# yukara-ikemiya/world-class

Measured on AMD Instinct MI355X. Metric: analysis+synthesis frames/sec (whole node), 48 kHz 5 ms hop, higher is better.
Workload: dtype f64; 1 GPU; 64 synthetic 48 kHz 10 s utterances per GPU (8 distinct, tiled), 5 ms hop, Harvest->CheapTrick->D4C->Synthesis, inputs resident in HBM when the clock starts (`value`; SURVEY.md section 8(d)'s headline with H2D of x and D2H of all outputs inside the clock is `value_with_transfers`); utterances_per_gpu=64, frames_per_gpu=128064, fs=48000, fft_size=2048, parallelism=utterance-sharded x1 (shard.partition), final RCCL all-gather of F0 + checksums

## Files before the change

### world_class_amd/csrc/wc_stages.hpp

```cpp
#pragma once
#include <utility>
#include <vector>

#include "wc_internal.hpp"
#include "wc_stretch.hpp"

inline bool fft_size_supported(int fft_size) { return fft_size == 512 || fft_size == 1024 || fft_size == 2048 || fft_size == 4096; }

int hv_enqueue(wc_harvest *h, hipStream_t s, int n_utt, const double *d_x, const int *x_length, double *d_tpos, double *d_f0,
			   bool full, hipEvent_t mid_event, hipEvent_t start_after, int part = 3, hipEvent_t bp_done = nullptr,
			   hipEvent_t tail_after = nullptr);
int hv_overflowed(wc_harvest *h, hipStream_t s, bool *overflow, bool *tie = nullptr, std::vector<int> *tie_utts = nullptr);
std::vector<std::pair<int, int>> hv_runs_of(const std::vector<int> &us);
wc_harvest *hv_exact_twin(wc_harvest *h);
void hv_set_phases(wc_harvest *h, int mask);
int hv_row_width(const wc_harvest *h);
int hv_reserve_rows(wc_harvest *h, long long total_1ms_frames);
double *hv_candidate_rows(wc_harvest *h);
double *hv_score_rows(wc_harvest *h);

int ct_prepare(wc_cheaptrick *c, hipStream_t s, int n_utt, const int *x_length, const double *d_f0, const int *f0_length,
			   const uint64_t *rng_pos, long long *total_out, uint64_t *min_pos_out, uint64_t *max_end_out);
int ct_frames(wc_cheaptrick *c, hipStream_t s, int n_utt, const double *d_x, const double *d_tpos, const double *d_f0,
			  double *d_sp, long long total, hipEvent_t *rows_done);
// ... 5 lines not shown
				const double *d_f0, const int *f0_length, int fft_size, double *d_ap, const uint64_t *rng_pos,
				const unsigned long long *d_start);
const unsigned long long *d4c_end_positions(const wc_d4c *d);
uint64_t d4c_draw_bound(const wc_d4c *d, int f0_length);

int syn_prepare(wc_synthesis *sy, hipStream_t s, int n_utt, const double *d_f0, const int *f0_length, const int *out_length,
				double *d_out, const uint64_t *rng_pos, bool full);
int syn_pulses(wc_synthesis *sy, hipStream_t s, const double *d_f0, const double *d_sp, const double *d_ap, double *d_out,
			   const unsigned long long *d_start);
int syn_finish(wc_synthesis *sy, hipStream_t s, uint64_t *rng_pos_out, bool *overflow);

wc::Device *hv_device(const wc_harvest *h);
wc::Device *ct_device(const wc_cheaptrick *c);
wc::Device *d4c_device(const wc_d4c *d);
wc::Device *syn_device(const wc_synthesis *sy);
const double *syn_dc_remover(const wc_synthesis *sy);
int syn_fs(const wc_synthesis *sy);

namespace wc {
struct CodecPlanArgs {
	const int *k;
	const double *s;
	const double2 *w;
};
struct CodecPlan {
	DevBuf k, s, w, kp, sp;
	CodecPlanArgs args() const { return {k.as<int>(), s.as<double>(), w.as<double2>()}; }
	CodecPlanArgs wave_args() const { return {kp.as<int>(), sp.as<double>(), w.as<double2>()}; }
};
int codec_plan(Device *dev, int fs, int fft_size, bool coding, const CodecPlan **out);
// ... 35 lines not shown
```

### world_class_amd/csrc/wc_synth_stream.hip

```cpp
#include <algorithm>
#include <cfloat>
#include <climits>
#include <cmath>
#include <cstring>
#include <vector>

#include "wc_stages.hpp"
#include "wc_synthesis.hpp"
#include "../../include/world_class_codec.h"
#include "../../include/world_class_stream.h"

namespace wc {

struct SsDesc {
	long long win_old, win_new;
	long long in_off;
	int keep_from, keep, n_in;
	int f_base, f_len;
	int n0, n1;
	int cap;
	int has_pend, pend_idx, pend_vuv;
	double pend_shift;
	double run, wrap, vu;
	long long inc_off, slot;
// ... 181 lines not shown
	bool formed = false;
	double last = 0.0;
	long long src = 0;
	int cside = 0;
};
}

struct wc_synth_stream {
	int fs, fft_size, n_streams, max_frames, fp_ms_x1000;
	double frame_period;
	int gap, wcap, ccap, wsz;
	Device *dev;
	wc_synthesis *sy;
	std::vector<SsState> st;
	int parity = 0;
	DevBuf wf0[2], wsp[2], wap[2], carry[2], work, inc, pulses, resp, meta, owner, aux;
	DevBuf dsp, dap;
	DevBuf dmod, sf0;
	DevBuf cf0, csp, cap, rf0, rsp, rap, drt;
	DevBuf tf0, tcsp, tcap;
	HostBuf h_stage, h_mod, h_rt;
};

namespace {
struct SynthStreamGuard {
	wc_synth_stream *s;
	std::vector<SsState> st;
	int parity;
	bool keep = false;
	explicit SynthStreamGuard(wc_synth_stream *x) : s(x), st(x->st), parity(x->parity) {}
	~SynthStreamGuard() {
// ... 83 lines not shown
	const double spf = s->frame_period * fs;
	s->wcap = max_frames_per_push + (int)std::ceil((s->gap + fft_size + 2.0 * spf) / spf) + 8;
	s->ccap = s->gap + fft_size + 64;
	s->wsz = (int)((max_frames_per_push + 2) * std::ceil(spf)) + s->gap + fft_size + 64;
	s->st.assign(n_streams, SsState());
	return s;
}

void wc_synth_stream_destroy(wc_synth_stream *s) {
	if (!s) return;
	s->dev->quiesce();
	for (int k = 0; k < 2; ++k) { s->wf0[k].release(); s->wsp[k].release(); s->wap[k].release(); s->carry[k].release(); }
	s->dsp.release(); s->dap.release(); s->dmod.release(); s->sf0.release(); s->h_mod.release();
	s->cf0.release(); s->csp.release(); s->cap.release(); s->rf0.release(); s->rsp.release(); s->rap.release(); s->drt.release(); s->h_rt.release();
	s->tf0.release(); s->tcsp.release(); s->tcap.release();
	s->work.release(); s->inc.release(); s->pulses.release(); s->resp.release(); s->meta.release(); s->owner.release(); s->aux.release(); s->h_stage.release();
	wc_synthesis_destroy(s->sy);
	delete s;
}

int wc_synth_stream_max_samples_per_push(const wc_synth_stream *s) { return s ? s->wsz : WC_ERR_INVALID; }

int wc_synth_stream_reset(wc_synth_stream *s, int u) {
	if (!s || u < 0 || u >= s->n_streams) return fail(WC_ERR_INVALID, "synthesis stream: bad stream index");
	DeviceLock lock(s->dev);
	s->st[u] = SsState();
	return WC_OK;
}

unsigned long long wc_synth_stream_rng_position(const wc_synth_stream *s, int u) {
	return (s && u >= 0 && u < s->n_streams) ? s->st[u].rng_pos : 0ull;
// ... 269 lines not shown
		SynArgs sa;
		std::memset(&sa, 0, sizeof(sa));
		sa.utts = d_utt; sa.n_utt = na; sa.pulse_prefix = d_prefix; sa.cap_off = d_capoff; sa.first_index = d_first; sa.p = pb;
		sa.f0 = s->wf0[1 - par].as<double>(); sa.sp = s->wsp[1 - par].as<double>(); sa.ap = s->wap[1 - par].as<double>();
		sa.tw = s->dev->twiddle; sa.dc_remover = syn_dc_remover(s->sy);
		sa.out = atomic ? s->work.as<double>() : nullptr;
		sa.resp = atomic ? nullptr : s->resp.as<double>();
		sa.rng_start = nullptr; sa.trace = nullptr; sa.only_pulse = -1; sa.fs = s->fs; sa.frame_period = s->frame_period;
		std::vector<int> owner((size_t)total_p);
		for (int a = 0; a < na; ++a) std::fill(owner.begin() + prefix[a], owner.begin() + prefix[a + 1], a);
		DevBuf &pu = s->owner;
		if ((rc = pu.reserve(sizeof(int) * (size_t)total_p * 2))) return rc;
		WC_HIP(hipMemcpyAsync(pu.p, owner.data(), sizeof(int) * (size_t)total_p, hipMemcpyHostToDevice, hs));
		WC_HIP(hipMemsetAsync(pu.as<int>() + total_p, 0, sizeof(int) * (size_t)total_p, hs));
		WC_HIP(hipStreamSynchronize(hs));
		if (atomic) {
			std::vector<OlDesc> ex(ol);
			for (auto &d : ex) { d.dst_off = d.src_off / s->ccap * s->wsz; d.cut = d.lo; }
			ol_expand = ex;
		}
		uint64_t lo = ~0ull, hi = 0;
		for (int a = 0; a < na; ++a) {
			if (n_syn[a] == 0) continue;
			lo = std::min<uint64_t>(lo, start[a]);
			hi = std::max<uint64_t>(hi, start[a] + (uint64_t)(E[act[a]] - first[a]) + 1);
		}
		if (atomic) {
			if ((rc = s->aux.reserve(sizeof(OlDesc) * na))) return rc;
			WC_HIP(hipMemcpyAsync(s->aux.p, ol_expand.data(), sizeof(OlDesc) * na, hipMemcpyHostToDevice, hs));
			overlap(nullptr, carry_old, s->work.as<double>(), s->aux.as<OlDesc>());
			WC_HIP(hipStreamSynchronize(hs));
		}
		if (hi - lo <= (1ull << 28)) {
			if ((rc = s->dev->ensure_rng(lo, hi))) return rc;
			sa.rng_table = s->dev->rng_table.as<uint32_t>(); sa.rng_base = s->dev->rng_base;
			sa.pulse_utt = pu.as<int>();
			sa.total_pulses = total_p;
			if ((rc = syn_launch_responses(N, sa, hs))) return rc;
		} else {
			for (int a = 0; a < na; ++a) {
				if (n_syn[a] == 0) continue;
				if ((rc = s->dev->ensure_rng(start[a], start[a] + (uint64_t)(E[act[a]] - first[a]) + 1))) return rc;
				SynArgs one = sa;
				one.utts = d_utt + a; one.n_utt = 1; one.pulse_prefix = d_pairs + 2 * a; one.cap_off = d_capoff + a; one.first_index = d_first + a;
				one.rng_table = s->dev->rng_table.as<uint32_t>(); one.rng_base = s->dev->rng_base;
				one.pulse_utt = pu.as<int>() + total_p;
				one.resp = atomic ? nullptr : s->resp.as<double>() + prefix[a] * N;
				one.total_pulses = n_syn[a];
				if ((rc = syn_launch_responses(N, one, hs))) return rc;
				WC_HIP(hipStreamSynchronize(hs));
			}
		}
	}
	if (atomic && total_p > 0) {
		std::vector<OlDesc> sp(ol);
		for (auto &d : sp) { d.src_off = d.src_off / s->ccap * s->wsz; d.src_len = d.hi - d.lo; d.n_p = 0; }
		if ((rc = s->h_stage.reserve(meta_bytes))) return rc;
		std::memcpy(s->h_stage.p, sp.data(), sizeof(OlDesc) * na);
		WC_HIP(hipMemcpyAsync(d_ol, s->h_stage.p, sizeof(OlDesc) * na, hipMemcpyHostToDevice, hs));
		if ((rc = s->h_stage.mark(hs))) return rc;
		overlap(nullptr, s->work.as<double>(), carry_new, d_ol);
	} else {
		overlap(atomic ? nullptr : s->resp.as<double>(), carry_old, carry_new, d_ol);
// ... 280 lines not shown
```

### world_class_amd/csrc/wc_synthesis.hip

```cpp
#include <cmath>
#include <cstdlib>
#include <cstring>
#include <vector>

#include "wc_device.hpp"
#include "wc_internal.hpp"
#include "wc_frames.hpp"
#include "wc_wavefft.hpp"
#include "wc_hostcopy.hpp"
#include "wc_synthesis.hpp"
#include "wc_stages.hpp"

namespace wc {

constexpr double kSafe = 0.000000000001;

struct TbArgs {
	const UttDesc *utts;
	const double *f0;
	const long long *cap_off;
	const int *cap;
	PulseBuf p;
	int *count;
	int *first_index;
// ... 1024 lines not shown
	wf_r2c_unpack(mr, mi, nyq, tw, lane);
#pragma unroll
	for (int s = 0; s < 16; ++s) {
		const double t = wf_exp_l(mr[s] * (0.5 / N), T);
		double sn, cs;
		wf_sincos(mi[s] * (0.5 / N), sn, cs);
		mr[s] = t * cs;
		mi[s] = t * sn;
	}
	mMr = wf_exp_l(nyq * (0.5 / N), T);
}

#ifndef WC_SYN_WAVE_OCC
#define WC_SYN_WAVE_OCC 2
#endif
#ifndef WC_SYN_ROWS_G
#define WC_SYN_ROWS_G 2
#endif
#ifndef WC_SYN_PARK_NOISE
#define WC_SYN_PARK_NOISE 1
#endif
#ifndef WC_SYN_ROW_PF
#define WC_SYN_ROW_PF 0
#endif
#ifndef WC_SYN_TRACE
#define WC_SYN_TRACE 0
#endif
#if WC_SYN_TRACE
#define SYN_STAMP(i) do { if (lane == 0) a.trace[gp * 16 + (i)] = __builtin_readcyclecounter(); } while (0)
#else
#define SYN_STAMP(i) do { } while (0)
#endif
template <bool ATOMIC>
__global__ __launch_bounds__(64) __attribute__((amdgpu_waves_per_eu(WC_SYN_WAVE_OCC, WC_SYN_WAVE_OCC))) void syn_pulse_wave_kernel(SynArgs a) {
	constexpr int N = 2048, M = 1024;
	__shared__ __attribute__((aligned(16))) double L[kWfLds];
	__shared__ __attribute__((aligned(16))) double T[kWfTabLds];
#if WC_SYN_PARK_NOISE
	__shared__ __attribute__((aligned(16))) double P[1024];
#endif
	const int lane = threadIdx.x;
#ifdef WC_SYN_LDS_PAD
	__shared__ double PAD[WC_SYN_LDS_PAD];
	if (a.fs < 0) PAD[lane] = 0.0;
#endif
	const long long total_p = a.pulse_prefix[a.n_utt];
	if ((long long)blockIdx.x >= 8 * ((total_p + 7) / 8)) return;
	const long long gp = xcd_frame(blockIdx.x, total_p);
	if (gp >= total_p) return;
	if (a.only_pulse >= 0 && gp != a.only_pulse) return;
	const int u = a.pulse_utt[gp];
	wf_tables_to_lds(T, a.tw, lane);
	const UttDesc ud = a.utts[u];
	const long long slot = a.cap_off[u] + (gp - a.pulse_prefix[u]);
	const int pidx = a.p.index[slot];
	const double shift = a.p.shift[slot];
	const int noise_size = a.p.noise_size[slot];
	const double vuv = (double)a.p.vuv[slot];
	const int fs = a.fs, Lf = ud.f_len;
	const double fp = a.frame_period;
	const double t = pidx / (double)fs;

	const int fl = min(Lf - 1, (int)floor(t / fp));
	const int ce = min(Lf - 1, (int)ceil(t / fp));
	const double ipol = uniform_d(t / fp - fl);
	const double *__restrict__ sf = a.sp + (ud.f_off + fl - ud.f_base) * (long long)(M + 1);
	const double *__restrict__ sc = a.sp + (ud.f_off + ce - ud.f_base) * (long long)(M + 1);
	const double *__restrict__ af = a.ap + (ud.f_off + fl - ud.f_base) * (long long)(M + 1);
	const double *__restrict__ ac = a.ap + (ud.f_off + ce - ud.f_base) * (long long)(M + 1);
	const bool same = fl == ce;
	auto blend = [&](double s0, double s1, double a0, double a1, double &env, double &ar) {
		if (same) {
			env = fabs(s0);
			const double s = safe_ap(a0);
			ar = s * s;
		} else {
			env = fma(1.0 - ipol, fabs(s0), ipol * fabs(s1));
			const double s = (1.0 - ipol) * safe_ap(a0) + ipol * safe_ap(a1);
			ar = s * s;
		}
	};
	double ar0;
	{
		double env;
		blend(sf[0], sc[0], af[0], ac[0], env, ar0);
		ar0 = uniform_d(ar0);
	}
#if WC_SYN_ROW_PF > 0
	double pf_s, pf_a;
	{
		const long long r2 = (ud.f_off + min(ce + WC_SYN_ROW_PF, Lf - 1) - ud.f_base) * (long long)(M + 1) + 16 * lane;
		pf_s = a.sp[r2];
		pf_a = a.ap[r2];
	}
#endif
	SYN_STAMP(0);
	SYN_STAMP(1);

	double dc = 0.0;
	const double sq = sqrt((double)noise_size);
#ifdef WC_SYN_RESP_ALIAS
	double *__restrict__ resp = a.resp + (gp & 2047) * (ATOMIC ? M : N);
#else
	double *__restrict__ resp = a.resp + gp * (ATOMIC ? M : N);
#endif
	double *__restrict__ yout = a.out + ud.y_off;
	const int ylen = ud.y_len;
	auto add2 = [&](int o, double v0, double v1) {
		if (o >= 0 && o < ylen) atomicAdd(yout + o, v0);
		if (o + 1 >= 0 && o + 1 < ylen) atomicAdd(yout + o + 1, v1);
	};
	const bool has_periodic = !(vuv <= 0.5 || ar0 > 0.999);
#pragma unroll 1
	for (int part = has_periodic ? 0 : 1; part < 2; ++part) {
		int ln = lane;
		WC_FRESH(ln);
		double wr[16], wi[16];
		double nr[16], ni[16], nsM = 0.0;
		if (part == 1) {
			const unsigned long long rstart = a.rng_start ? a.rng_start[u] : ud.rng_pos;
			const uint32_t *__restrict__ rng = a.rng_table + (rstart + (unsigned long long)(pidx - a.first_index[u]) - a.rng_base);
			double s = 0.0;
			{
				uint32_t raw[32];
#pragma unroll
				for (int q = 0; q < 16; ++q) {
					if ((q & 3) == 0 && q * 128 >= noise_size) break;
					const int i0 = 2 * ln + 128 * q;
					raw[2 * q] = rng[i0 < noise_size ? i0 : 0];
					raw[2 * q + 1] = rng[i0 + 1 < noise_size ? i0 + 1 : 0];
				}
				WF_SCHED_FENCE();
#pragma unroll
				for (int q = 0; q < 16; ++q) {
					nr[q] = ni[q] = 0.0;
					if (q * 128 < ((noise_size + 511) & ~511)) {
						const int i0 = 2 * ln + 128 * q;
						if (i0 < noise_size) nr[q] = raw[2 * q] / 268435456.0 - 6.0;
						if (i0 + 1 < noise_size) ni[q] = raw[2 * q + 1] / 268435456.0 - 6.0;
						s += nr[q] + ni[q];
					}
				}
			}
			s = wave_sum_all(s);
			const double avg = s / noise_size;
#pragma unroll
			for (int q = 0; q < 16; ++q) {
				const int i0 = 2 * ln + 128 * q;
				nr[q] = (i0 < noise_size) ? nr[q] - avg : 0.0;
				ni[q] = (i0 + 1 < noise_size) ? ni[q] - avg : 0.0;
			}
			if (noise_size <= 512) wdft16<+1, 1>(nr, ni);
			else if (noise_size <= 1024) wdft16<+1, 2>(nr, ni);
			else wdft16<+1, 4>(nr, ni);
			wf_fft1024_dit_rest<+1>(nr, ni, L, a.tw, ln);
			wf_r2c_unpack(nr, ni, nsM, a.tw, ln);
			SYN_STAMP(6);
#if WC_SYN_PARK_NOISE
#pragma unroll
			for (int sI = 0; sI < 16; ++sI) {
				P[64 * sI + ln] = nr[sI];
				resp[64 * sI + ln] = ni[sI];
			}
			wf_fence();
#endif
		}
		double mM;
		{
			auto logspec = [&](double env, double ar) {
				return wf_log_l(part == 0 ? env * (1.0 - ar) + kSafe : (vuv != 0.0 ? env * ar : env), T) / 2.0;
			};
#pragma unroll
			for (int g0 = 0; g0 < 4; g0 += WC_SYN_ROWS_G) {
				double v[4 * WC_SYN_ROWS_G][4];
#pragma unroll
				for (int q = 0; q < 4 * WC_SYN_ROWS_G; ++q) {
					const int k = wf_bin(ln, g0 + (q >> 2), q & 3);
					v[q][0] = sf[k]; v[q][1] = sc[k]; v[q][2] = af[k]; v[q][3] = ac[k];
				}
				WF_SCHED_FENCE();
#pragma unroll
				for (int q = 0; q < 4 * WC_SYN_ROWS_G; ++q) {
					double env, ar;
					blend(v[q][0], v[q][1], v[q][2], v[q][3], env, ar);
					L[wf_bin(ln, g0 + (q >> 2), q & 3)] = logspec(env, ar);
				}
			}
			double env, ar;
			blend(sf[M], sc[M], af[M], ac[M], env, ar);
			const double lsM = logspec(env, ar);
			if (ln == 0) L[M] = lsM;
		}
		SYN_STAMP(part ? 7 : 2);
		minimum_phase_wave(wr, wi, mM, L, T, a.tw, ln);
		SYN_STAMP(part ? 8 : 3);
		double yM;
		if (part == 0) {
			const double coef = 2.0 * kPi * shift * fs / N;
#pragma unroll
			for (int g = 0; g < 4; ++g)
#pragma unroll
				for (int q = 0; q < 4; ++q) {
					const int k = wf_bin(ln, g, q);
					double sn_, re2;
					wf_sincos(coef * k, sn_, re2);
					const double im2 = sqrt(1.0 - re2 * re2);
					const double x = wr[4 * g + q], y = wi[4 * g + q];
					wr[4 * g + q] = fma(x, re2, -(y * im2));
					wi[4 * g + q] = fma(x, im2, y * re2);
				}
			double sn_, reM;
			wf_sincos(coef * M, sn_, reM);
			yM = mM * reM;
		} else {
#if WC_SYN_PARK_NOISE
			{
				const double *rp = resp;
				asm volatile("" : "+s"(rp));
#pragma unroll
				for (int sI = 0; sI < 16; ++sI) {
					ni[sI] = rp[64 * sI + ln];
					nr[sI] = P[64 * sI + ln];
				}
				WF_SCHED_FENCE();
			}
#endif
#pragma unroll
			for (int sI = 0; sI < 16; ++sI) {
				const double x = wr[sI], y = wi[sI], nx = 0.5 * nr[sI], ny = 0.5 * ni[sI];
				wr[sI] = fma(x, nx, -(y * ny));
				wi[sI] = fma(x, ny, y * nx);
			}
			yM = mM * (0.5 * nsM);
		}
		wf_c2r_pack(wr, wi, yM, a.tw, ln);
		wf_fft1024_dif<-1>(wr, wi, L, a.tw, ln);
		SYN_STAMP(part ? 9 : 4);
// ... 12 lines not shown
		} else {
			const double dcs = has_periodic ? -dc * sq : 0.0;
			if (ATOMIC) {
#pragma unroll
				for (int q0 = 0; q0 < 8; q0 += 4) {
					double2 dr[4];
#pragma unroll
					for (int q = 0; q < 4; ++q) dr[q] = *reinterpret_cast<const double2 *>(a.dc_remover + 2 * ln + 128 * (q0 + q));
					WF_SCHED_FENCE();
#pragma unroll
					for (int q = 0; q < 4; ++q) {
						const int n = 2 * ln + 128 * (q0 + q);
						add2(pidx + 1 + n, fma(dcs, dr[q].x, wr[q0 + q]) / N, fma(dcs, dr[q].y, wi[q0 + q]) / N);
						add2(pidx + 1 - M + n, fma(dcs, dr[q].x, wr[q0 + q + 8]) / N, fma(dcs, dr[q].y, wi[q0 + q + 8]) / N);
					}
				}
			} else
#pragma unroll
			for (int q0 = 0; q0 < 8; q0 += 4) {
				double2 dr[4], pp[4];
#pragma unroll
				for (int q = 0; q < 4; ++q) {
					dr[q] = *reinterpret_cast<const double2 *>(a.dc_remover + 2 * ln + 128 * (q0 + q));
					pp[q] = has_periodic ? *reinterpret_cast<const double2 *>(resp + M + 2 * ln + 128 * (q0 + q)) : make_double2(0.0, 0.0);
				}
				WF_SCHED_FENCE();
#pragma unroll
				for (int q = 0; q < 4; ++q) {
					const int n = 2 * ln + 128 * (q0 + q);
					const double r0 = fma(dcs, dr[q].x, wr[q0 + q]) + pp[q].x, r1 = fma(dcs, dr[q].y, wi[q0 + q]) + pp[q].y;
// ... 264 lines not shown
				const double r0 = fma(dcs, dr[q].x, wr[q]) + pp[q].x, r1 = fma(dcs, dr[q].y, wi[q]) + pp[q].y;
				*reinterpret_cast<double2 *>(resp + n + M) = make_double2(r0 / N, r1 / N);
				const double r2 = fma(dcs, dr[q].x, wr[q + 4]), r3 = fma(dcs, dr[q].y, wi[q + 4]);
				*reinterpret_cast<double2 *>(resp + n) = make_double2(r2 / N, r3 / N);
			}
		}
	}
}

__global__ void syn_pulse_utt_kernel(const long long *__restrict__ prefix, int *__restrict__ pulse_utt) {
	const int u = blockIdx.x;
	const long long lo = prefix[u], hi = prefix[u + 1];
	for (long long g = lo + threadIdx.x; g < hi; g += blockDim.x) pulse_utt[g] = u;
}

constexpr int OA_T = 256, OA_K = 4, OA_TILE = OA_T * OA_K;
template <int N>
__global__ __launch_bounds__(OA_T) void syn_overlap_add_kernel(SynArgs a) {
	constexpr int M = N / 2;
	const int u = blockIdx.y;
	const UttDesc ud = a.utts[u];
	const int t0 = blockIdx.x * OA_TILE;
	if (t0 >= ud.y_len) return;
	const long long pre = a.pulse_prefix[u];
	const int n_p = (int)(a.pulse_prefix[u + 1] - pre);
	const int *__restrict__ pidx = a.p.index + a.cap_off[u];
	int lo = 0, hi = n_p;
	while (lo < hi) {
		const int mid = (lo + hi) >> 1;
		if (pidx[mid] < t0 - M) lo = mid + 1; else hi = mid;
// ... 32 lines not shown
	}
}

}

using namespace wc;

struct wc_synthesis {
	int fs, fft_size;
	double frame_period;
	Device *dev;
	wc_synthesis *twin = nullptr;
	hipStream_t s_twin = nullptr;
	hipEvent_t e_twin = nullptr;
	bool is_twin = false;
	DevBuf dc_remover, utts, meta, pulses, incs, phase, phase_seg, tile_cnt, resp, pulse_utt, d_f0, d_sp, d_ap, d_out;
	bool pulses_by_utterance;
	bool wave;
	bool rows = false;
	bool wave_atomic = false;
	size_t rows_budget = 0;
	bool phase_single;
	bool serial_timebase;
	HostBuf h_stage, h_rows;
	DevBuf dec_sp, dec_ap;
	DevBuf rt_f0, rt_sp, rt_ap;
	long long total_out = 0, cap_total = 0;
	int n_utt = 0, max_out = 0;
};

template <int N>
static void launch_pulses(const SynArgs &a, hipStream_t s) {
	constexpr int TP = (N >= 2048) ? 256 : (N / 8 < 64 ? 64 : N / 8);
	hipLaunchKernelGGL((syn_pulse_kernel<N, TP>), dim3((unsigned)(8 * ((a.total_pulses + 7) / 8))), dim3(TP), 0, s, a);
}

int wc::syn_launch_responses(int fft_size, const SynArgs &a, hipStream_t s) {
	switch (fft_size) {
		case 512: launch_pulses<512>(a, s); break;
		case 1024: {
			const long long per = (a.total_pulses + 7) / 8;
			hipLaunchKernelGGL(syn_pulse_wave8_kernel, dim3((unsigned)(8 * ((per + kSyn8Waves - 1) / kSyn8Waves))), dim3(64 * kSyn8Waves), 0, s, a);
			break;
		}
		case 2048: hipLaunchKernelGGL(syn_pulse_wave_kernel<false>, dim3((unsigned)(8 * ((a.total_pulses + 7) / 8))), dim3(64), 0, s, a); break;
		case 4096: launch_pulses<4096>(a, s); break;
		default: return fail(WC_ERR_UNSUPPORTED, "synthesis: fft_size must be 512, 1024, 2048 or 4096");
	}
	WC_HIP(hipGetLastError());
	return WC_OK;
}

__global__ void syn_prefix_kernel(int n_utt, const int *__restrict__ count, const int *__restrict__ cap,
								  const int *__restrict__ first_index, const int *__restrict__ last_index,
								  const UttDesc *__restrict__ utts, const unsigned long long *__restrict__ d_start,
								  long long *__restrict__ prefix, unsigned long long *__restrict__ end_pos, int *__restrict__ overflow) {
	if (threadIdx.x != 0) return;
	long long run = 0;
	int ovf = 0;
	for (int u = 0; u < n_utt; ++u) {
		prefix[u] = run;
		if (count[u] > cap[u]) ovf = 1;
		run += min(count[u], cap[u]);
		const unsigned long long st = d_start ? d_start[u] : utts[u].rng_pos;
// ... 148 lines not shown
	a.first_index = d_first; a.p = pb; a.f0 = d_f0; a.sp = d_sp; a.ap = d_ap;
	a.rng_table = dev->rng_table.as<uint32_t>(); a.rng_base = dev->rng_base; a.tw = dev->twiddle;
	a.dc_remover = sy->dc_remover.as<double>(); a.out = d_out; a.total_pulses = co; a.fs = sy->fs;
	a.frame_period = sy->frame_period; a.rng_start = d_start;
#ifdef WC_DEBUG_HOOKS
	{
		const char *dbg = getenv("WC_DEBUG_ONLY_PULSE");
		a.only_pulse = dbg ? atoll(dbg) : -1;
	}
#else
	a.only_pulse = -1;
#endif
	a.trace = nullptr;
	a.resp = nullptr;
	a.pulse_utt = nullptr;
	if (sy->rows) {
		const bool atomic_rows = sy->wave_atomic && sy->fft_size == 2048;
		if ((rc = sy->resp.reserve(sizeof(double) * (size_t)(atomic_rows ? sy->fft_size / 2 : sy->fft_size) * (size_t)co))) return rc;
		a.resp = sy->resp.as<double>();
		if ((rc = sy->pulse_utt.reserve(sizeof(int) * (size_t)co))) return rc;
		a.pulse_utt = sy->pulse_utt.as<int>();
		hipLaunchKernelGGL(syn_pulse_utt_kernel, dim3(n_utt), dim3(256), 0, s, (const long long *)d_prefix, sy->pulse_utt.as<int>());
	}
#if WC_SYN_TRACE
	static DevBuf tracebuf;
	if (tracebuf.reserve(sizeof(unsigned long long) * 16 * (size_t)co)) return WC_ERR_DEVICE;
	(void)hipMemsetAsync(tracebuf.p, 0, sizeof(unsigned long long) * 16 * (size_t)co, s);
	a.trace = tracebuf.as<unsigned long long>();
#endif
	if ((rc = dev->time_begin("synthesis_pulses", s))) return rc;
	switch (sy->fft_size) {
		case 512: launch_pulses<512>(a, s); break;
		case 1024:
			if (sy->rows) {
				const long long per = (a.total_pulses + 7) / 8;
				hipLaunchKernelGGL(syn_pulse_wave8_kernel, dim3((unsigned)(8 * ((per + kSyn8Waves - 1) / kSyn8Waves))), dim3(64 * kSyn8Waves), 0, s, a);
				hipLaunchKernelGGL(syn_overlap_add_kernel<1024>, dim3((unsigned)((sy->max_out + OA_TILE - 1) / OA_TILE), n_utt), dim3(OA_T), 0, s, a);
			} else {
				launch_pulses<1024>(a, s);
			}
			break;
		case 2048:
			if (sy->rows) {
				if (sy->wave_atomic) {
					hipLaunchKernelGGL(syn_pulse_wave_kernel<true>, dim3((unsigned)(8 * ((a.total_pulses + 7) / 8))), dim3(64), 0, s, a);
				} else {
					hipLaunchKernelGGL(syn_pulse_wave_kernel<false>, dim3((unsigned)(8 * ((a.total_pulses + 7) / 8))), dim3(64), 0, s, a);
					hipLaunchKernelGGL(syn_overlap_add_kernel<2048>, dim3((unsigned)((sy->max_out + OA_TILE - 1) / OA_TILE), n_utt), dim3(OA_T), 0, s, a);
				}
			} else {
				launch_pulses<2048>(a, s);
			}
			break;
		case 4096: launch_pulses<4096>(a, s); break;
		default: return fail(WC_ERR_UNSUPPORTED, "synthesis: fft_size must be 512, 1024, 2048 or 4096");
	}
	WC_HIP(hipGetLastError());
#if WC_SYN_TRACE
	if (const char *path = getenv("WC_SYN_TRACE_FILE")) {
		std::vector<unsigned long long> h((size_t)16 * co);
		WC_HIP(hipStreamSynchronize(s));
		WC_HIP(hipMemcpy(h.data(), a.trace, sizeof(unsigned long long) * h.size(), hipMemcpyDeviceToHost));
// ... 86 lines not shown
		return fail(WC_ERR_DEVICE, "synthesis: pulse buffer overflow");
	}
	for (int attempt = 0; attempt < 2; ++attempt) {
		if ((rc = syn_prepare(sy, s, n_utt, d_f0, f0_length, out_length, d_out, rng_pos, attempt == 1))) return rc;
		if ((rc = syn_pulses(sy, s, d_f0, d_sp, d_ap, d_out, nullptr))) return rc;
		bool overflow = false;
		if ((rc = syn_finish(sy, s, rng_pos, &overflow))) return rc;
		if (!overflow) return WC_OK;
	}
	return fail(WC_ERR_DEVICE, "synthesis: pulse buffer overflow");
}

wc::Device *syn_device(const wc_synthesis *sy) { return sy->dev; }
int syn_fs(const wc_synthesis *sy) { return sy->fs; }
const double *syn_dc_remover(const wc_synthesis *sy) { return sy->dc_remover.as<double>(); }

extern "C" {

wc_synthesis *wc_synthesis_create(int fs, int fft_size, double frame_period_ms) {
	if (fs <= 0 || frame_period_ms <= 0) { set_error("synthesis: fs and frame_period must be positive"); return nullptr; }
	if (!fft_size_supported(fft_size)) {
		set_error("synthesis: fft_size must be 512, 1024, 2048 or 4096");
		return nullptr;
	}
	Device *dev = current_device();
	if (!dev) return nullptr;
	wc_synthesis *s = new wc_synthesis();
	s->fs = fs;
	s->fft_size = fft_size;
	s->frame_period = frame_period_ms / 1000.;
	{
		const char *tb = getenv("WC_SYN_TIMEBASE");
		s->serial_timebase = tb && std::string(tb) == "serial";
		const char *ph = getenv("WC_SYN_PHASE");
		s->phase_single = ph && std::string(ph) == "single";
		const char *pu = getenv("WC_SYN_PULSES");
		s->pulses_by_utterance = pu && std::string(pu) == "utterance";
		const char *impl = getenv("WC_SYN_IMPL");
		s->wave = !(impl && std::string(impl) == "block");
		const char *ola = getenv("WC_SYN_OLA");
		s->wave_atomic = ola && std::string(ola) == "atomic";
		size_t free_b = 0, total_b = 0;
		if (hipMemGetInfo(&free_b, &total_b) != hipSuccess) total_b = (size_t)64 << 30;
		s->rows_budget = total_b / 8;
		if (const char *mb = getenv("WC_SYN_ROWS_BUDGET_MB")) s->rows_budget = (size_t)atoll(mb) << 20;
	}
	s->dev = dev;
	std::vector<double> d(fft_size);
	const double cv = 2.0 * 3.1415926535897932384 / (1.0 + fft_size);
	for (int i = 0; i < fft_size / 2; ++i) d[i] = 0.5 - 0.5 * std::cos(cv * (i + 1.0));
	double dc = 0.0;
	for (int i = 0; i < fft_size / 2; ++i) dc += d[i];
	dc *= 2;
	for (int i = 0; i < fft_size / 2; ++i) { d[i] /= dc; d[fft_size - i - 1] = d[i]; }
	if (s->dc_remover.reserve(sizeof(double) * fft_size) ||
		hipMemcpy(s->dc_remover.p, d.data(), sizeof(double) * fft_size, hipMemcpyHostToDevice) != hipSuccess) {
		set_error("synthesis: table upload failed");
		delete s;
		return nullptr;
	}
	dev->handle_born();
	return s;
}
void wc_synthesis_destroy(wc_synthesis *s) {
	if (!s) return;
	s->dev->quiesce();
	s->dev->handle_gone();
	if (s->twin) wc_synthesis_destroy(s->twin);
	if (s->s_twin) (void)hipStreamDestroy(s->s_twin);
	if (s->e_twin) (void)hipEventDestroy(s->e_twin);
	s->dc_remover.release(); s->utts.release(); s->meta.release(); s->pulses.release(); s->incs.release(); s->phase.release(); s->tile_cnt.release(); s->phase_seg.release(); s->resp.release(); s->pulse_utt.release();
	s->d_f0.release(); s->d_sp.release(); s->d_ap.release(); s->d_out.release(); s->h_stage.release(); s->h_rows.release();
	s->dec_sp.release(); s->dec_ap.release();
	s->rt_f0.release(); s->rt_sp.release(); s->rt_ap.release();
	delete s;
}

int wc_synthesis_get_fft_size(const wc_synthesis *s) { return s ? s->fft_size : WC_ERR_INVALID; }

int wc_synthesis_compute_device(wc_synthesis *s, int n_utt, const double *d_f0, const int *f0_length, const double *d_sp,
								const double *d_ap, const int *out_length, double *d_out, uint64_t *rng_pos) {
	if (!s || n_utt <= 0 || !d_f0 || !f0_length || !d_sp || !d_ap || !out_length || !d_out)
		return fail(WC_ERR_INVALID, "synthesis: null argument");
	WC_HIP(hipSetDevice(s->dev->id));
	DeviceLock lock(s->dev);
	return syn_run_device(s, n_utt, d_f0, f0_length, d_sp, d_ap, out_length, d_out, rng_pos);
// ... 99 lines not shown
```

### world_class_amd/csrc/wc_synthesis.hpp

```cpp
#pragma once
#include <cstdint>

#include "wc_device.hpp"
#include "wc_internal.hpp"

namespace wc {

struct PulseBuf {
	int *index;
	double *shift;
	int *noise_size;
	int *vuv;
};

struct Coarse {
	const double *f0;
	int L;
	double lowest_f0, fp;
	int base = 0;
	__device__ __forceinline__ double cf_in(int j) const {
		double v = f0[j - base];
		return (v < lowest_f0) ? 0.0 : v;
	}
	__device__ __forceinline__ double cv_in(int j) const { return (cf_in(j) == 0.0) ? 0.0 : 1.0; }
// ... 107 lines not shown

struct SynArgs {
	const UttDesc *utts;
	int n_utt;
	const long long *pulse_prefix;
	const long long *cap_off;
	const int *first_index;
	PulseBuf p;
	const double *f0, *sp, *ap;
	const uint32_t *rng_table;
	unsigned long long rng_base;
	const double2 *tw;
	const double *dc_remover;
	double *out;
	const int *pulse_utt;
	double *resp;
	long long total_pulses;
	const unsigned long long *rng_start;
	unsigned long long *trace;
	long long only_pulse;
	int fs;
	double frame_period;
};

int syn_launch_responses(int fft_size, const SynArgs &a, hipStream_t s);

}
```

Before: 5.123 million frames/s.

## Split synthesis pulses into voiced and unvoiced classes with specialized wave kernels

Adds a class-listing pass that partitions pulses into voiced and unvoiced index lists. Two specialized instantiations of the 2048-point pulse wave kernel then run over them. The unvoiced kernel skips the periodic part and aperiodicity blending, handles short noise with a single-slot path instead of the full DFT, and can use separate occupancy tuning. The voiced kernel can compute the noise log-spectrum row during the periodic pass. The cost is two extra small kernels, an extra launch, and more code paths, in exchange for less divergent, lighter per-pulse work.

```diff
diff --git a/world_class_amd/csrc/wc_stages.hpp b/world_class_amd/csrc/wc_stages.hpp
--- a/world_class_amd/csrc/wc_stages.hpp
+++ b/world_class_amd/csrc/wc_stages.hpp
@@ -43,6 +43,7 @@
 wc::Device *ct_device(const wc_cheaptrick *c);
 wc::Device *d4c_device(const wc_d4c *d);
 wc::Device *syn_device(const wc_synthesis *sy);
+bool syn_split(const wc_synthesis *sy);
 const double *syn_dc_remover(const wc_synthesis *sy);
 int syn_fs(const wc_synthesis *sy);
 
diff --git a/world_class_amd/csrc/wc_synth_stream.hip b/world_class_amd/csrc/wc_synth_stream.hip
--- a/world_class_amd/csrc/wc_synth_stream.hip
+++ b/world_class_amd/csrc/wc_synth_stream.hip
@@ -219,7 +219,7 @@
 	wc_synthesis *sy;
 	std::vector<SsState> st;
 	int parity = 0;
-	DevBuf wf0[2], wsp[2], wap[2], carry[2], work, inc, pulses, resp, meta, owner, aux;
+	DevBuf wf0[2], wsp[2], wap[2], carry[2], work, inc, pulses, resp, meta, owner, aux, cls;
 	DevBuf dsp, dap;
 	DevBuf dmod, sf0;
 	DevBuf cf0, csp, cap, rf0, rsp, rap, drt;
@@ -333,7 +333,7 @@
 	s->dsp.release(); s->dap.release(); s->dmod.release(); s->sf0.release(); s->h_mod.release();
 	s->cf0.release(); s->csp.release(); s->cap.release(); s->rf0.release(); s->rsp.release(); s->rap.release(); s->drt.release(); s->h_rt.release();
 	s->tf0.release(); s->tcsp.release(); s->tcap.release();
-	s->work.release(); s->inc.release(); s->pulses.release(); s->resp.release(); s->meta.release(); s->owner.release(); s->aux.release(); s->h_stage.release();
+	s->work.release(); s->inc.release(); s->pulses.release(); s->resp.release(); s->meta.release(); s->owner.release(); s->aux.release(); s->cls.release(); s->h_stage.release();
 	wc_synthesis_destroy(s->sy);
 	delete s;
 }
@@ -633,6 +633,8 @@
 		WC_HIP(hipMemcpyAsync(pu.p, owner.data(), sizeof(int) * (size_t)total_p, hipMemcpyHostToDevice, hs));
 		WC_HIP(hipMemsetAsync(pu.as<int>() + total_p, 0, sizeof(int) * (size_t)total_p, hs));
 		WC_HIP(hipStreamSynchronize(hs));
+		const bool split = N == 2048 && !atomic && syn_split(s->sy);
+		if (split && (rc = s->cls.reserve(sizeof(int) * syn_class_ints(total_p, na)))) return rc;
 		if (atomic) {
 			std::vector<OlDesc> ex(ol);
 			for (auto &d : ex) { d.dst_off = d.src_off / s->ccap * s->wsz; d.cut = d.lo; }
@@ -655,6 +657,7 @@
 			sa.rng_table = s->dev->rng_table.as<uint32_t>(); sa.rng_base = s->dev->rng_base;
 			sa.pulse_utt = pu.as<int>();
 			sa.total_pulses = total_p;
+			if (split && (rc = syn_launch_class_lists(sa, s->cls.as<int>(), nullptr, hs))) return rc;
 			if ((rc = syn_launch_responses(N, sa, hs))) return rc;
 		} else {
 			for (int a = 0; a < na; ++a) {
@@ -666,6 +669,7 @@
 				one.pulse_utt = pu.as<int>() + total_p;
 				one.resp = atomic ? nullptr : s->resp.as<double>() + prefix[a] * N;
 				one.total_pulses = n_syn[a];
+				if (split && (rc = syn_launch_class_lists(one, s->cls.as<int>(), nullptr, hs))) return rc;
 				if ((rc = syn_launch_responses(N, one, hs))) return rc;
 				WC_HIP(hipStreamSynchronize(hs));
 			}
diff --git a/world_class_amd/csrc/wc_synthesis.hip b/world_class_amd/csrc/wc_synthesis.hip
--- a/world_class_amd/csrc/wc_synthesis.hip
+++ b/world_class_amd/csrc/wc_synthesis.hip
@@ -1062,6 +1062,9 @@
 #ifndef WC_SYN_WAVE_OCC
 #define WC_SYN_WAVE_OCC 2
 #endif
+#ifndef WC_SYN_UNV_OCC
+#define WC_SYN_UNV_OCC 2
+#endif
 #ifndef WC_SYN_ROWS_G
 #define WC_SYN_ROWS_G 2
 #endif
@@ -1079,9 +1082,12 @@
 #else
 #define SYN_STAMP(i) do { } while (0)
 #endif
-template <bool ATOMIC>
-__global__ __launch_bounds__(64) __attribute__((amdgpu_waves_per_eu(WC_SYN_WAVE_OCC, WC_SYN_WAVE_OCC))) void syn_pulse_wave_kernel(SynArgs a) {
+template <bool ATOMIC, int CLS = 0>
+__global__ __launch_bounds__(64) __attribute__((amdgpu_waves_per_eu(CLS == 2 ? WC_SYN_UNV_OCC : WC_SYN_WAVE_OCC, CLS == 2 ? WC_SYN_UNV_OCC : WC_SYN_WAVE_OCC)))
+void syn_pulse_wave_kernel(SynArgs a) {
 	constexpr int N = 2048, M = 1024;
+	constexpr bool kRowsOnce = CLS == 1 && WC_SYN_PARK_NOISE;
+	constexpr bool kParkRow = CLS == 2 && WC_SYN_UNV_OCC > 2 && !ATOMIC;
 	__shared__ __attribute__((aligned(16))) double L[kWfLds];
 	__shared__ __attribute__((aligned(16))) double T[kWfTabLds];
 #if WC_SYN_PARK_NOISE
@@ -1092,10 +1098,11 @@
 	__shared__ double PAD[WC_SYN_LDS_PAD];
 	if (a.fs < 0) PAD[lane] = 0.0;
 #endif
-	const long long total_p = a.pulse_prefix[a.n_utt];
+	const long long total_p = CLS == 0 ? a.pulse_prefix[a.n_utt] : (long long)a.cls_count[CLS - 1];
 	if ((long long)blockIdx.x >= 8 * ((total_p + 7) / 8)) return;
-	const long long gp = xcd_frame(blockIdx.x, total_p);
-	if (gp >= total_p) return;
+	const long long place = xcd_frame(blockIdx.x, total_p);
+	if (place >= total_p) return;
+	const long long gp = CLS == 0 ? place : (long long)a.cls_list[(CLS - 1) * a.total_pulses + place];
 	if (a.only_pulse >= 0 && gp != a.only_pulse) return;
 	const int u = a.pulse_utt[gp];
 	wf_tables_to_lds(T, a.tw, lane);
@@ -1104,7 +1111,7 @@
 	const int pidx = a.p.index[slot];
 	const double shift = a.p.shift[slot];
 	const int noise_size = a.p.noise_size[slot];
-	const double vuv = (double)a.p.vuv[slot];
+	const double vuv = CLS == 0 ? (double)a.p.vuv[slot] : (CLS == 1 ? 1.0 : 0.0);
 	const int fs = a.fs, Lf = ud.f_len;
 	const double fp = a.frame_period;
 	const double t = pidx / (double)fs;
@@ -1128,8 +1135,9 @@
 			ar = s * s;
 		}
 	};
-	double ar0;
-	{
+	auto blend_env = [&](double s0, double s1) { return same ? fabs(s0) : fma(1.0 - ipol, fabs(s0), ipol * fabs(s1)); };
+	double ar0 = 1.0;
+	if constexpr (CLS != 2) {
 		double env;
 		blend(sf[0], sc[0], af[0], ac[0], env, ar0);
 		ar0 = uniform_d(ar0);
@@ -1158,9 +1166,10 @@
 		if (o >= 0 && o < ylen) atomicAdd(yout + o, v0);
 		if (o + 1 >= 0 && o + 1 < ylen) atomicAdd(yout + o + 1, v1);
 	};
-	const bool has_periodic = !(vuv <= 0.5 || ar0 > 0.999);
+	const bool has_periodic = CLS != 2 && !(vuv <= 0.5 || ar0 > 0.999);
+	const int part_first = (CLS == 2 || !has_periodic) ? 1 : 0;
 #pragma unroll 1
-	for (int part = has_periodic ? 0 : 1; part < 2; ++part) {
+	for (int part = part_first; part < 2; ++part) {
 		int ln = lane;
 		WC_FRESH(ln);
 		double wr[16], wi[16];
@@ -1168,8 +1177,16 @@
 		if (part == 1) {
 			const unsigned long long rstart = a.rng_start ? a.rng_start[u] : ud.rng_pos;
 			const uint32_t *__restrict__ rng = a.rng_table + (rstart + (unsigned long long)(pidx - a.first_index[u]) - a.rng_base);
+			const bool slot0_only = CLS == 2 && noise_size <= 128;
 			double s = 0.0;
-			{
+			if (slot0_only) {
+				const int i0 = 2 * ln;
+				const uint32_t raw0 = rng[i0 < noise_size ? i0 : 0], raw1 = rng[i0 + 1 < noise_size ? i0 + 1 : 0];
+				nr[0] = ni[0] = 0.0;
+				if (i0 < noise_size) nr[0] = raw0 / 268435456.0 - 6.0;
+				if (i0 + 1 < noise_size) ni[0] = raw1 / 268435456.0 - 6.0;
+				s += nr[0] + ni[0];
+			} else {
 				uint32_t raw[32];
 #pragma unroll
 				for (int q = 0; q < 16; ++q) {
@@ -1192,32 +1209,65 @@
 			}
 			s = wave_sum_all(s);
 			const double avg = s / noise_size;
-#pragma unroll
-			for (int q = 0; q < 16; ++q) {
-				const int i0 = 2 * ln + 128 * q;
-				nr[q] = (i0 < noise_size) ? nr[q] - avg : 0.0;
-				ni[q] = (i0 + 1 < noise_size) ? ni[q] - avg : 0.0;
-			}
-			if (noise_size <= 512) wdft16<+1, 1>(nr, ni);
-			else if (noise_size <= 1024) wdft16<+1, 2>(nr, ni);
-			else wdft16<+1, 4>(nr, ni);
+			if (slot0_only) {
+				const int i0 = 2 * ln;
+				nr[0] = (i0 < noise_size) ? nr[0] - avg : 0.0;
+				ni[0] = (i0 + 1 < noise_size) ? ni[0] - avg : 0.0;
+#pragma unroll
+				for (int q = 1; q < 16; ++q) { nr[q] = nr[0]; ni[q] = ni[0]; }
+			} else {
+#pragma unroll
+				for (int q = 0; q < 16; ++q) {
+					const int i0 = 2 * ln + 128 * q;
+					nr[q] = (i0 < noise_size) ? nr[q] - avg : 0.0;
+					ni[q] = (i0 + 1 < noise_size) ? ni[q] - avg : 0.0;
+				}
+				if (noise_size <= 512) wdft16<+1, 1>(nr, ni);
+				else if (noise_size <= 1024) wdft16<+1, 2>(nr, ni);
+				else wdft16<+1, 4>(nr, ni);
+			}
 			wf_fft1024_dit_rest<+1>(nr, ni, L, a.tw, ln);
 			wf_r2c_unpack(nr, ni, nsM, a.tw, ln);
 			SYN_STAMP(6);
 #if WC_SYN_PARK_NOISE
+			const bool swap = kRowsOnce && has_periodic;
+			if (swap) wf_fence();
 #pragma unroll
 			for (int sI = 0; sI < 16; ++sI) {
-				P[64 * sI + ln] = nr[sI];
+				if constexpr (kParkRow) {
+					resp[M + 64 * sI + ln] = nr[sI];
+				} else {
+					if (swap) L[64 * sI + ln] = P[64 * sI + ln];
+					P[64 * sI + ln] = nr[sI];
+				}
 				resp[64 * sI + ln] = ni[sI];
 			}
+			if (swap && ln == 0) L[M] = L[kWfLds - 1];
 			wf_fence();
 #endif
 		}
 		double mM;
-		{
+		if constexpr (CLS == 2) {
+#pragma unroll
+			for (int g0 = 0; g0 < 4; g0 += WC_SYN_ROWS_G) {
+				double v[4 * WC_SYN_ROWS_G][2];
+#pragma unroll
+				for (int q = 0; q < 4 * WC_SYN_ROWS_G; ++q) {
+					const int k = wf_bin(ln, g0 + (q >> 2), q & 3);
+					v[q][0] = sf[k]; v[q][1] = sc[k];
+				}
+				WF_SCHED_FENCE();
+#pragma unroll
+				for (int q = 0; q < 4 * WC_SYN_ROWS_G; ++q)
+					L[wf_bin(ln, g0 + (q >> 2), q & 3)] = wf_log_l(blend_env(v[q][0], v[q][1]), T) / 2.0;
+			}
+			const double lsM = wf_log_l(blend_env(sf[M], sc[M]), T) / 2.0;
+			if (ln == 0) L[M] = lsM;
+		} else if (!kRowsOnce || part == part_first) {
 			auto logspec = [&](double env, double ar) {
 				return wf_log_l(part == 0 ? env * (1.0 - ar) + kSafe : (vuv != 0.0 ? env * ar : env), T) / 2.0;
 			};
+			const bool both = kRowsOnce && part == 0;
 #pragma unroll
 			for (int g0 = 0; g0 < 4; g0 += WC_SYN_ROWS_G) {
 				double v[4 * WC_SYN_ROWS_G][4];
@@ -1232,12 +1282,19 @@
 					double env, ar;
 					blend(v[q][0], v[q][1], v[q][2], v[q][3], env, ar);
 					L[wf_bin(ln, g0 + (q >> 2), q & 3)] = logspec(env, ar);
+#if WC_SYN_PARK_NOISE
+					if (both) P[wf_bin(ln, g0 + (q >> 2), q & 3)] = wf_log_l(env * ar, T) / 2.0;
+#endif
 				}
 			}
 			double env, ar;
 			blend(sf[M], sc[M], af[M], ac[M], env, ar);
 			const double lsM = logspec(env, ar);
 			if (ln == 0) L[M] = lsM;
+			if (both) {
+				const double lsM1 = wf_log_l(env * ar, T) / 2.0;
+				if (ln == 0) L[kWfLds - 1] = lsM1;
+			}
 		}
 		SYN_STAMP(part ? 7 : 2);
 		minimum_phase_wave(wr, wi, mM, L, T, a.tw, ln);
@@ -1268,7 +1325,8 @@
 #pragma unroll
 				for (int sI = 0; sI < 16; ++sI) {
 					ni[sI] = rp[64 * sI + ln];
-					nr[sI] = P[64 * sI + ln];
+					if constexpr (kParkRow) nr[sI] = rp[M + 64 * sI + ln];
+					else nr[sI] = P[64 * sI + ln];
 				}
 				WF_SCHED_FENCE();
 			}
@@ -1311,6 +1369,13 @@
 						add2(pidx + 1 + n, fma(dcs, dr[q].x, wr[q0 + q]) / N, fma(dcs, dr[q].y, wi[q0 + q]) / N);
 						add2(pidx + 1 - M + n, fma(dcs, dr[q].x, wr[q0 + q + 8]) / N, fma(dcs, dr[q].y, wi[q0 + q + 8]) / N);
 					}
+				}
+			} else if constexpr (CLS == 2) {
+#pragma unroll
+				for (int q = 0; q < 8; ++q) {
+					const int n = 2 * ln + 128 * q;
+					*reinterpret_cast<double2 *>(resp + n + M) = make_double2(wr[q] / N, wi[q] / N);
+					*reinterpret_cast<double2 *>(resp + n) = make_double2(wr[q + 8] / N, wi[q + 8] / N);
 				}
 			} else
 #pragma unroll
@@ -1605,6 +1670,71 @@
 	for (long long g = lo + threadIdx.x; g < hi; g += blockDim.x) pulse_utt[g] = u;
 }
 
+constexpr int CL_T = 256;
+__global__ __launch_bounds__(CL_T) void syn_class_count_kernel(const long long *__restrict__ prefix, const long long *__restrict__ cap_off,
+															   const int *__restrict__ vuv, int *__restrict__ pulse_utt, int *__restrict__ voiced) {
+	__shared__ int tot;
+	const int u = blockIdx.x;
+	const long long lo = prefix[u];
+	const int n = (int)(prefix[u + 1] - lo);
+	const int *__restrict__ v = vuv + cap_off[u];
+	if (threadIdx.x == 0) tot = 0;
+	__syncthreads();
+	int c = 0;
+	for (int i = threadIdx.x; i < n; i += CL_T) {
+		c += v[i] != 0;
+		if (pulse_utt) pulse_utt[lo + i] = u;
+	}
+	if (c) atomicAdd(&tot, c);
+	__syncthreads();
+	if (threadIdx.x == 0) voiced[u] = tot;
+}
+__global__ __launch_bounds__(CL_T) void syn_class_lists_kernel(int n_utt, const long long *__restrict__ prefix, const long long *__restrict__ cap_off,
+															   const int *__restrict__ vuv, const int *__restrict__ voiced, long long cap,
+															   int *__restrict__ list, int *__restrict__ count) {
+	__shared__ int front, all, wv[CL_T / 64];
+	const int u = blockIdx.x, tid = threadIdx.x, w = tid >> 6;
+	const long long lo = prefix[u];
+	const int n = (int)(prefix[u + 1] - lo);
+	const int *__restrict__ v = vuv + cap_off[u];
+	if (tid == 0) front = all = 0;
+	__syncthreads();
+	{
+		int f = 0, t = 0;
+		for (int k = tid; k < n_utt; k += CL_T) {
+			const int c = voiced[k];
+			t += c;
+			if (k < u) f += c;
+		}
+		if (f) atomicAdd(&front, f);
+		if (t) atomicAdd(&all, t);
+	}
+	__syncthreads();
+	if (u == 0 && tid == 0) {
+		count[0] = all;
+		count[1] = (int)(prefix[n_utt] - all);
+	}
+	long long at_v = front, at_u = cap + (lo - front);
+	for (int base = 0; base < n; base += CL_T) {
+		const int i = base + tid;
+		const bool in = i < n, vo = in && v[i] != 0;
+		const unsigned long long b = __ballot(vo);
+		if ((tid & 63) == 0) wv[w] = __popcll(b);
+		__syncthreads();
+		int rank = __popcll(b & ((1ull << (tid & 63)) - 1ull)), chunk_v = 0;
+#pragma unroll
+		for (int k = 0; k < CL_T / 64; ++k) {
+			if (k < w) rank += wv[k];
+			chunk_v += wv[k];
+		}
+		if (vo) list[at_v + rank] = (int)(lo + i);
+		else if (in) list[at_u + (tid - rank)] = (int)(lo + i);
+		at_v += chunk_v;
+		at_u += CL_T - chunk_v;
+		__syncthreads();
+	}
+}
+
 constexpr int OA_T = 256, OA_K = 4, OA_TILE = OA_T * OA_K;
 template <int N>
 __global__ __launch_bounds__(OA_T) void syn_overlap_add_kernel(SynArgs a) {
@@ -1667,11 +1797,12 @@
 	hipStream_t s_twin = nullptr;
 	hipEvent_t e_twin = nullptr;
 	bool is_twin = false;
-	DevBuf dc_remover, utts, meta, pulses, incs, phase, phase_seg, tile_cnt, resp, pulse_utt, d_f0, d_sp, d_ap, d_out;
+	DevBuf dc_remover, utts, meta, pulses, incs, phase, phase_seg, tile_cnt, resp, pulse_utt, cls, d_f0, d_sp, d_ap, d_out;
 	bool pulses_by_utterance;
 	bool wave;
 	bool rows = false;
 	bool wave_atomic = false;
+	bool split = true;
 	size_t rows_budget = 0;
 	bool phase_single;
 	bool serial_timebase;
@@ -1688,6 +1819,16 @@
 	hipLaunchKernelGGL((syn_pulse_kernel<N, TP>), dim3((unsigned)(8 * ((a.total_pulses + 7) / 8))), dim3(TP), 0, s, a);
 }
 
+static void launch_pulse_waves(const SynArgs &a, hipStream_t s) {
+	const dim3 grid((unsigned)(8 * ((a.total_pulses + 7) / 8)));
+	if (a.cls_list) {
+		hipLaunchKernelGGL((syn_pulse_wave_kernel<false, 1>), grid, dim3(64), 0, s, a);
+		hipLaunchKernelGGL((syn_pulse_wave_kernel<false, 2>), grid, dim3(64), 0, s, a);
+	} else {
+		hipLaunchKernelGGL((syn_pulse_wave_kernel<false, 0>), grid, dim3(64), 0, s, a);
+	}
+}
+
 int wc::syn_launch_responses(int fft_size, const SynArgs &a, hipStream_t s) {
 	switch (fft_size) {
 		case 512: launch_pulses<512>(a, s); break;
@@ -1696,11 +1837,23 @@
 			hipLaunchKernelGGL(syn_pulse_wave8_kernel, dim3((unsigned)(8 * ((per + kSyn8Waves - 1) / kSyn8Waves))), dim3(64 * kSyn8Waves), 0, s, a);
 			break;
 		}
-		case 2048: hipLaunchKernelGGL(syn_pulse_wave_kernel<false>, dim3((unsigned)(8 * ((a.total_pulses + 7) / 8))), dim3(64), 0, s, a); break;
+		case 2048: launch_pulse_waves(a, s); break;
 		case 4096: launch_pulses<4096>(a, s); break;
 		default: return fail(WC_ERR_UNSUPPORTED, "synthesis: fft_size must be 512, 1024, 2048 or 4096");
 	}
 	WC_HIP(hipGetLastError());
+	return WC_OK;
+}
+
+size_t wc::syn_class_ints(long long total_pulses, int n_utt) { return 2 * (size_t)total_pulses + 2 + (size_t)n_utt; }
+int wc::syn_launch_class_lists(SynArgs &a, int *buf, int *pulse_utt, hipStream_t s) {
+	int *count = buf + 2 * a.total_pulses, *voiced = count + 2;
+	hipLaunchKernelGGL(syn_class_count_kernel, dim3(a.n_utt), dim3(CL_T), 0, s, a.pulse_prefix, a.cap_off, (const int *)a.p.vuv, pulse_utt, voiced);
+	hipLaunchKernelGGL(syn_class_lists_kernel, dim3(a.n_utt), dim3(CL_T), 0, s, a.n_utt, a.pulse_prefix, a.cap_off, (const int *)a.p.vuv,
+					   (const int *)voiced, a.total_pulses, buf, count);
+	WC_HIP(hipGetLastError());
+	a.cls_list = buf;
+	a.cls_count = count;
 	return WC_OK;
 }
 
@@ -1879,13 +2032,19 @@
 	a.trace = nullptr;
 	a.resp = nullptr;
 	a.pulse_utt = nullptr;
+	a.cls_list = a.cls_count = nullptr;
 	if (sy->rows) {
 		const bool atomic_rows = sy->wave_atomic && sy->fft_size == 2048;
 		if ((rc = sy->resp.reserve(sizeof(double) * (size_t)(atomic_rows ? sy->fft_size / 2 : sy->fft_size) * (size_t)co))) return rc;
 		a.resp = sy->resp.as<double>();
 		if ((rc = sy->pulse_utt.reserve(sizeof(int) * (size_t)co))) return rc;
 		a.pulse_utt = sy->pulse_utt.as<int>();
-		hipLaunchKernelGGL(syn_pulse_utt_kernel, dim3(n_utt), dim3(256), 0, s, (const long long *)d_prefix, sy->pulse_utt.as<int>());
+		if (sy->split && sy->fft_size == 2048 && !sy->wave_atomic) {
+			if ((rc = sy->cls.reserve(sizeof(int) * syn_class_ints(co, n_utt)))) return rc;
+			if ((rc = syn_launch_class_lists(a, sy->cls.as<int>(), sy->pulse_utt.as<int>(), s))) return rc;
+		} else {
+			hipLaunchKernelGGL(syn_pulse_utt_kernel, dim3(n_utt), dim3(256), 0, s, (const long long *)d_prefix, sy->pulse_utt.as<int>());
+		}
 	}
 #if WC_SYN_TRACE
 	static DevBuf tracebuf;
@@ -1910,7 +2069,7 @@
 				if (sy->wave_atomic) {
 					hipLaunchKernelGGL(syn_pulse_wave_kernel<true>, dim3((unsigned)(8 * ((a.total_pulses + 7) / 8))), dim3(64), 0, s, a);
 				} else {
-					hipLaunchKernelGGL(syn_pulse_wave_kernel<false>, dim3((unsigned)(8 * ((a.total_pulses + 7) / 8))), dim3(64), 0, s, a);
+					launch_pulse_waves(a, s);
 					hipLaunchKernelGGL(syn_overlap_add_kernel<2048>, dim3((unsigned)((sy->max_out + OA_TILE - 1) / OA_TILE), n_utt), dim3(OA_T), 0, s, a);
 				}
 			} else {
@@ -2027,6 +2186,7 @@
 wc::Device *syn_device(const wc_synthesis *sy) { return sy->dev; }
 int syn_fs(const wc_synthesis *sy) { return sy->fs; }
 const double *syn_dc_remover(const wc_synthesis *sy) { return sy->dc_remover.as<double>(); }
+bool syn_split(const wc_synthesis *sy) { return sy->split; }
 
 extern "C" {
 
@@ -2053,6 +2213,8 @@
 		s->wave = !(impl && std::string(impl) == "block");
 		const char *ola = getenv("WC_SYN_OLA");
 		s->wave_atomic = ola && std::string(ola) == "atomic";
+		const char *sp = getenv("WC_SYN_SPLIT");
+		s->split = !(sp && sp[0] == '0');
 		size_t free_b = 0, total_b = 0;
 		if (hipMemGetInfo(&free_b, &total_b) != hipSuccess) total_b = (size_t)64 << 30;
 		s->rows_budget = total_b / 8;
@@ -2082,7 +2244,7 @@
 	if (s->twin) wc_synthesis_destroy(s->twin);
 	if (s->s_twin) (void)hipStreamDestroy(s->s_twin);
 	if (s->e_twin) (void)hipEventDestroy(s->e_twin);
-	s->dc_remover.release(); s->utts.release(); s->meta.release(); s->pulses.release(); s->incs.release(); s->phase.release(); s->tile_cnt.release(); s->phase_seg.release(); s->resp.release(); s->pulse_utt.release();
+	s->dc_remover.release(); s->utts.release(); s->meta.release(); s->pulses.release(); s->incs.release(); s->phase.release(); s->tile_cnt.release(); s->phase_seg.release(); s->resp.release(); s->pulse_utt.release(); s->cls.release();
 	s->d_f0.release(); s->d_sp.release(); s->d_ap.release(); s->d_out.release(); s->h_stage.release(); s->h_rows.release();
 	s->dec_sp.release(); s->dec_ap.release();
 	s->rt_f0.release(); s->rt_sp.release(); s->rt_ap.release();
diff --git a/world_class_amd/csrc/wc_synthesis.hpp b/world_class_amd/csrc/wc_synthesis.hpp
--- a/world_class_amd/csrc/wc_synthesis.hpp
+++ b/world_class_amd/csrc/wc_synthesis.hpp
@@ -145,6 +145,7 @@
 	const double *dc_remover;
 	double *out;
 	const int *pulse_utt;
+	const int *cls_list, *cls_count;
 	double *resp;
 	long long total_pulses;
 	const unsigned long long *rng_start;
@@ -155,5 +156,7 @@
 };
 
 int syn_launch_responses(int fft_size, const SynArgs &a, hipStream_t s);
+size_t syn_class_ints(long long total_pulses, int n_utt);
+int syn_launch_class_lists(SynArgs &a, int *buf, int *pulse_utt, hipStream_t s);
 
 }
```

Result: faster. 5.195 million frames/s, median of 6 (+1.4%).
